# HybridRobotics/ilqr-iterative-tasks

Measured on AMD Instinct MI355X. Metric: batched iLQR iterations/s (n=6,m=2,N=20), higher is better.
Workload: dtype f64

## Files before the change

ilqr_iterative_tasks_amd/csrc/i2lqr_abi.hip:

```cpp
#include <hip/hip_runtime.h>

#include <atomic>
#include <cmath>
#include <cstdarg>
#include <cstdio>
#include <cstdlib>
#include <cstring>
#include <mutex>
#include <new>
#include <unordered_set>

#include "../../include/i2lqr.h"
#include "i2lqr_devcfg.hpp"
#include "i2lqr_geometry.hpp"
#include "i2lqr_group.h"
#include "i2lqr_handle.hpp"
#include "i2lqr_host.hpp"
#include "i2lqr_kernels.h"
#include "i2lqr_lane12.h"
#include "i2lqr_rccl.hpp"
#include "i2lqr_select.hpp"
#include "i2lqr_wave_opt.h"

#include "i2lqr_lane_launch.hpp"
// ... 499 lines not shown
  else if (!strcmp(name, "merge_inputs")) lane.opt_merge = v < 0 ? -1 : (v != 0);
  else if (!strcmp(name, "checkpoint_states")) lane.opt_ckpt = v < 0 ? -1 : (v != 0);
  else if (!strcmp(name, "stagger")) lane.opt_stagger = v;
  else if (!strcmp(name, "per_step_jacobians")) col.opt_fstep = v < 0 ? -1 : (v != 0);
  else if (!strcmp(name, "wave_tail")) lane.wave_tail = v < 0 ? -1 : (v > 65536 ? 65536 : v);
  else if (!strcmp(name, "first_chunk")) lane.opt_first_chunk = v < 1 ? -1 : (v > 1024 ? 1024 : v);
  else if (!strcmp(name, "helper_wavefront")) lane.opt_pair = v < 0 ? -1 : (v != 0);
  else if (!strcmp(name, "state_buffers")) lane.opt_two_x = v < 0 ? -1 : (v != 0);
  else if (!strcmp(name, "chunk_step")) lane.opt_chunk_step = v < 1 ? -1 : (v > 1024 ? 1024 : v);
  else if (!strcmp(name, "fused_compaction")) lane.opt_fuse = v < 0 ? -1 : (v != 0);
  else if (!strcmp(name, "final_round")) lane.opt_final_round = v < 0 ? -1 : (v > 20 ? 20 : v);
  else if (!strcmp(name, "speculate")) col.opt_spec = v < 0 ? -1 : (v != 0);
  else if (!strcmp(name, "group_workspace")) col.opt_group_ws = v < 0 ? -1 : (v != 0);
  else if (!strcmp(name, "group_overlap")) col.opt_group_overlap = v < 0 ? -1 : (v != 0);
  else if (!strcmp(name, "group_fixed_horizon")) col.opt_group_fixed = v < 0 ? -1 : (v != 0);
  else if (!strcmp(name, "debug_self_test")) {
#ifdef I2LQR_DEBUG
    unsigned long long* w = i2lqr::debug_trap_word();
    double* buf = nullptr;
    HIP_TRY(hipMalloc((void**)&buf, 8 * sizeof(double)));
    hipLaunchKernelGGL(k_debug_self_test, dim3(1), dim3(64), 0, (hipStream_t)0, buf, w);
    const int rc = debug_check(I2LQR_OK, nullptr);
    (void)hipFree(buf);
    return rc;
#else
    return fail(I2LQR_ERR_UNSUPPORTED, "\"debug_self_test\" exists in the index-checked debug build "
                "only (make -C ilqr_iterative_tasks_amd/csrc debug)");
#endif
  }
  else if (!strcmp(name, "line_search")) {
// ... 601 lines not shown
```

ilqr_iterative_tasks_amd/csrc/i2lqr_column_launch.hpp:

```cpp
#pragma once
#include <hip/hip_runtime.h>

#include "i2lqr_column_plan.hpp"
#include "i2lqr_devcfg.hpp"
#include "i2lqr_group.h"
#include "i2lqr_handle.hpp"
#include "i2lqr_host.hpp"
#include "i2lqr_kernels.h"
#include "i2lqr_wave_opt.h"

namespace i2lqr {

inline thread_local i2lqr_handle::Epilogue* t_epi = nullptr;

inline int64_t registered_ws(const i2lqr_handle* h) { return h->ws ? h->ws_bytes : -1; }
inline ColumnChoice column_kernel(const i2lqr_handle* h, int64_t B, bool early_exit) {
  return column_kernel(h->geo, h->fit, h->col, h->model.form(), registered_ws(h), B, early_exit);
}

inline int wave_lds_check(const i2lqr_handle* h, bool chained) {
  const size_t need = wave_lds_need(h->fit, h->model, chained);
  if (need <= h->geo.max_dyn_lds) return I2LQR_OK;
  const WaveForm f = h->model.form(chained);
  const int n_obs = h->model.records();
// ... 23 lines not shown
      return fail(I2LQR_ERR_UNSUPPORTED, "horizon %d needs %zu B of LDS per wavefront (> %zu KiB)",
                  h->cfg.N, lds, h->geo.max_dyn_lds / 1024);
    if (lds > h->geo.default_dyn_lds)
      for (const void* kernel :
           {(const void*)k_iterate<T, Sys, LANES, false>, (const void*)k_iterate<T, Sys, LANES, true>,
            (const void*)k_backward<T, Sys, LANES, false>, (const void*)k_backward<T, Sys, LANES, true>,
            (const void*)k_forward<T, Sys, LANES, false>, (const void*)k_forward<T, Sys, LANES, true>,
            (const void*)k_rollout<T, Sys, LANES, false>, (const void*)k_rollout<T, Sys, LANES, true>})
        HIP_TRY(hipFuncSetAttribute(kernel, hipFuncAttributeMaxDynamicSharedMemorySize, (int)lds));
    return I2LQR_OK;
  }

  static int iterate(i2lqr_handle* h, const SolveIO& io, hipStream_t s) {
    const int64_t B = io.B;
    IterArgs<T> a = iter_args<T>(io);
#ifdef I2LQR_STAMPS
    a.dbg = (unsigned long long*)h->ws;
#endif
    const ColumnChoice choice = column_kernel(h, B, io.early_exit != 0);
    const ColumnKernel fk = choice.kernel;
    if (t_epi && (fk == K_GROUP || fk == K_GROUP16 || fk == K_GROUP_WS)) {
      a.qfun = t_epi->qfun;
      a.outer_iter = t_epi->outer_iter;
      a.max_relax_iter = t_epi->max_relax_iter;
      a.cost_it = (T*)t_epi->cost_it;
      if (t_epi->best_idx) {
        a.pick_part = (MinPair<T>*)t_epi->part;
        a.pick_ticket = h->ticket + h->ticket_next.fetch_add(1, std::memory_order_relaxed) %
                                        i2lqr_handle::kTickets;
        a.best_idx = t_epi->best_idx;
// ... 62 lines not shown
        return I2LQR_OK;
      }
    }
    with_weights(c.flags, [&](auto W) {
      hipLaunchKernelGGL((k_iterate<T, Sys, LANES, W>), dim3(grid(B)), dim3(64), h->fit.lds_wave, s, c, a);
    });
    HIP_TRY(hipGetLastError());
    return I2LQR_OK;
  }
  static int names_pair(const i2lqr_handle*, int64_t, int) { return 0; }
  static int solve_chained(i2lqr_handle* h, const SolveIO& io, int k, hipStream_t s) {
    const ChainPlan plan = chain_plan(h->geo, h->fit, h->col, h->model.form(), registered_ws(h), io.B);
    if (plan.kind == ChainPlan::REFUSED) return fail(I2LQR_ERR_UNSUPPORTED, "%s", plan.why);
    IterArgs<T> a = iter_args<T>(io);
    a.chain_len = k;
    if (plan.kind == ChainPlan::WAVE) {
      if (int rc = wave_lds_check(h, true)) return rc;
      HIP_TRY(wave_opt_launch<T>(h->cfg, a, h->model, true, h->fit.lds_wave, s));
    } else if constexpr (kBicycle) {
      HIP_TRY(group_spec_chain<T>(h->cfg, a, s));
    }
    return I2LQR_OK;
  }
  static int rollout(i2lqr_handle* h, int64_t B, void* X, void* U, const void* x_term, void* cost,
                     hipStream_t s) {
    const Cfg c = make_dev_cfg<T, n, m>(h->cfg);
    with_weights(c.flags, [&](auto W) {
      hipLaunchKernelGGL((k_rollout<T, Sys, LANES, W>), dim3(grid(B)), dim3(64), h->fit.lds_wave, s, c,
                         B, (T*)X, (T*)U, (const T*)x_term, (T*)cost);
    });
// ... 30 lines not shown
```

ilqr_iterative_tasks_amd/csrc/i2lqr_column_plan.hpp:

```cpp
#pragma once
#include <cstddef>
#include <cstdint>
#include <cstdio>

#include "../../include/i2lqr.h"
#include "i2lqr_geometry.hpp"
#include "i2lqr_wave_model.hpp"

namespace i2lqr {

struct ColumnTune {
  int opt_fstep = -1;
  int opt_group = -1;
  int opt_spec = -1;
  int opt_group_ws = -1;
  int opt_group_overlap = -1;
  int opt_group_fixed = -1;
  int opt_wave_chain = 0;
};

struct ColumnFit {
  enum Plant { OTHER, BICYCLE, SIXTEEN };
  int plant = OTHER;
  bool weights = false;
  bool problem_major = false;
  bool f64 = true;
  int n = 0, N = 0, word = 8;
  bool fixed_horizon = false;
  size_t lds_wave = 0, lds_wave_fstep = 0;
  size_t lds_group8 = 0, lds_group16 = 0;
  size_t lds_group_ws = 0;
  size_t lds_spec8x2 = 0, lds_spec8x3 = 0;
// ... 243 lines not shown
```

ilqr_iterative_tasks_amd/csrc/i2lqr_dryrun.hpp:

```cpp
#pragma once
#ifdef I2LQR_DRY_RUN
#include <hip/hip_runtime.h>

#include <cstddef>
#include <cstdint>

#include "i2lqr_wave.hpp"

namespace i2lqr {
namespace dry {

bool on();
void allow(const void* base, size_t bytes);
void reset();
void record(const char* expr, const void* kernel, dim3 grid, dim3 block, size_t lds);
void ptr(const char* field, const void* p);
void val(const char* field, int64_t v);
void end();
int64_t report(char* buf, int64_t n);

template <class A> inline void arg(const A&) {}
inline void arg(int64_t v) { val("int", v); }
inline void arg(int v) { val("int", v); }
template <class P> inline void arg(P* p) { ptr("pointer argument", (const void*)p); }
// ... 4 lines not shown
  ptr("IterArgs.K", a.K); ptr("IterArgs.k", a.k); ptr("IterArgs.iters", a.iters);
  ptr("IterArgs.status", a.status); ptr("IterArgs.dbg", a.dbg); ptr("IterArgs.count", a.count);
  val("IterArgs.count_max", a.count_max); val("IterArgs.max_total", a.max_total);
  val("IterArgs.set_stride", a.set_stride);
  ptr("IterArgs.orig", a.orig); ptr("IterArgs.out_X", a.out_X);
  ptr("IterArgs.out_U", a.out_U); ptr("IterArgs.out_K", a.out_K);
  ptr("IterArgs.out_k", a.out_k); ptr("IterArgs.out_lamb", a.out_lamb);
  ptr("IterArgs.out_cost", a.out_cost); ptr("IterArgs.out_iters", a.out_iters);
  ptr("IterArgs.out_status", a.out_status);
  val("IterArgs.out_B", a.out_B); val("IterArgs.out_tiled", a.out_tiled);
  ptr("IterArgs.qfun", a.qfun);
  val("IterArgs.outer_iter", a.outer_iter); val("IterArgs.max_relax_iter", a.max_relax_iter);
  ptr("IterArgs.cost_it", a.cost_it); ptr("IterArgs.pick_part", a.pick_part);
  ptr("IterArgs.pick_ticket", a.pick_ticket); ptr("IterArgs.best_idx", a.best_idx);
  ptr("IterArgs.best_cost", a.best_cost); val("IterArgs.chain_len", a.chain_len);
}
#ifdef I2LQR_DRY_RUN_LANE
template <class T> inline void arg(const LaneSet<T>& s) {
  ptr("LaneSet.X", s.X); ptr("LaneSet.U", s.U); ptr("LaneSet.x_term", s.x_term);
  ptr("LaneSet.obs", s.obs); ptr("LaneSet.lamb", s.lamb); ptr("LaneSet.cost", s.cost);
  ptr("LaneSet.K", s.K); ptr("LaneSet.k", s.k); ptr("LaneSet.iters", s.iters);
  ptr("LaneSet.status", s.status); ptr("LaneSet.orig", s.orig); val("LaneSet.B", s.B);
}
template <class T> inline void arg(const LaneArgs<T>& a) {
  val("LaneArgs.B", a.B); val("LaneArgs.n_iters", a.n_iters); val("LaneArgs.early_exit", a.early_exit);
  ptr("LaneArgs.X", a.X); ptr("LaneArgs.U", a.U); ptr("LaneArgs.x_term", a.x_term);
  ptr("LaneArgs.lamb", a.lamb); ptr("LaneArgs.obs", a.obs); ptr("LaneArgs.cost", a.cost);
  ptr("LaneArgs.K", a.K); ptr("LaneArgs.k", a.k); ptr("LaneArgs.iters", a.iters);
  ptr("LaneArgs.status", a.status); ptr("LaneArgs.wsU", a.wsU); ptr("LaneArgs.wsK", a.wsK);
  ptr("LaneArgs.wsk", a.wsk); ptr("LaneArgs.wsX", a.wsX); ptr("LaneArgs.count", a.count);
// ... 48 lines not shown
```

ilqr_iterative_tasks_amd/csrc/i2lqr_group.hpp:

```cpp
#pragma once
#include <hip/hip_runtime.h>
#include <stdint.h>

#include "i2lqr_systems.hpp"
#include "i2lqr_wave.hpp"

namespace i2lqr {

constexpr int kGroup = 8;
constexpr int kGroupsPerWave = 64 / kGroup;

template <class Sys> struct GroupPattern {
  static constexpr int n = Sys::n, m = Sys::m, W = n + m, NV = Sys::NVAR;
  static constexpr int dt_row(int b) {
    for (int i = 2; i < n; i++)
      if (i != b && Sys::pat(i, b) == 2) return i;
    return -1;
  }
  static constexpr bool column_ok(int b) {
    int extra = 0;
    for (int i = 0; i < n; i++) {
      const int code = Sys::pat(i, b);
      if (i < 2) {
        if (code == 2) return false;
// ... 206 lines not shown
  template <int i, int a> __device__ __forceinline__ void f_acc(T& acc, bool& first, T v,
                                                                const T (&jv)[NV]) const {
    constexpr int code = Sys::pat(i, a);
    if constexpr (code == 0) {
      return;
    } else if constexpr (code == 1) {
      acc = first ? v : acc + v;
      first = false;
    } else {
      const T f = code == 2 ? c.dt : jv[code >= 3 ? code - 3 : 0];
      acc = first ? f * v : t_fma(f, v, acc);
      first = false;
    }
  }

  __device__ __forceinline__ T rollout(int XUo, int TRo, const T (&xT)[n]) const {
    T x[n], u[m], xn[n], tr[NT];
#pragma unroll
    for (int i = 0; i < n; i++) x[i] = S[XUo + i];
    const int N = loop_N();
    for (int t = 0; t < N; t++) {
#pragma unroll
      for (int a = 0; a < m; a++) u[a] = clip(S[XUo + t * W + n + a], -c.u_max[a], c.u_max[a]);
#pragma unroll
      for (int a = 0; a < m; a++) S[XUo + t * W + n + a] = u[a];
      Sys::trig(x, tr);
#pragma unroll
      for (int q = 0; q < NT; q++) S[TRo + t * NT + q] = tr[q];
      Sys::step_tr(c, x, u, tr, xn);
#pragma unroll
      for (int i = 0; i < n; i++) S[XUo + (t + 1) * W + i] = xn[i];
#pragma unroll
      for (int i = 0; i < n; i++) x[i] = xn[i];
    }
    Sys::trig(x, tr);
#pragma unroll
    for (int q = 0; q < NT; q++) S[TRo + N * NT + q] = tr[q];
    const T cost = terminal_cost(x, xT);
    wave_sync();
    return cost;
  }

  __device__ __forceinline__ void prep(int XUo, int TRo, const T (&ob)[6], T pa, T pb, int first,
                                       int stride) const {
    const bool has_ob = ob[5] >= T(0);
    const int opt = has_ob ? (int)ob[5] : 0;
    const T spd_y = opt == 1 ? ob[4] : T(0), spd_x = opt == 2 ? ob[4] : T(0);
    const int rounds = (N + stride) / stride;
    for (int r = 0; r < rounds; r++) {
      const int t0 = first + r * stride;
      const int t = t0 < N ? t0 : N;
      const int ts = t0 < N ? t0 : N - 1;
      T* Rs = rec(ts);
      {
        T xe[n], tr[NT], u[m], jv[NV];
#pragma unroll
        for (int i = 0; i < n; i++) xe[i] = S[XUo + (ts + 1) * W + i];
#pragma unroll
        for (int a = 0; a < m; a++) u[a] = S[XUo + ts * W + n + a];
// ... 21 lines not shown
      R[GL::R_ZERO] = T(0);
      R[GL::R_ONE] = T(1);
      const T px = S[XUo + t * W + 0], py = S[XUo + t * W + 1];
      const T dz = opt == 2 ? px - (ob[0] - T(t) * spd_x) : px - ob[0];
      const T dy = opt == 1 ? py - (ob[1] + T(t) * spd_y) : py - ob[1];
      const T h = T(1) + c.safety_margin - (dz * pa * dz + dy * pb * dy);
      const T hd0 = T(-2) * pa * dz, hd1 = T(-2) * pb * dy;
      const T e = t_exp(c.obs_q2 * h);
      const T c1 = c.obs_q12 * e, c2 = c.obs_q122 * e;
      R[GL::R_OB + 0] = has_ob ? c1 * hd0 : T(0);
      R[GL::R_OB + 1] = has_ob ? c1 * hd1 : T(0);
      R[GL::R_OB + 2] = has_ob ? c2 * (hd0 * hd0) : T(0);
      R[GL::R_OB + 3] = has_ob ? c2 * (hd0 * hd1) : T(0);
      R[GL::R_OB + 4] = has_ob ? c2 * (hd1 * hd1) : T(0);
    }
    wave_sync();
    ws_publish();
  }

  __device__ __forceinline__ void quu_inverse(const T (&Quu)[m * m], T lamb, T (&inv)[m * m]) const {
    static_assert(m == 2, "the eight-lane kernel is written for m == 2 plants");
    t_quu_inverse2(Quu, lamb, inv);
  }

  template <bool GENERAL>
  __device__ __forceinline__ bool backward(int XUo, const T (&xT)[n], T lamb, bool commit) const {
    if constexpr (G == 16) return backward_row<GENERAL>(XUo, xT, lamb, commit);
    bool bad = false;
    T va[n];
    {
      const T* Rn = rec(N);
      T dx[n];
// ... 346 lines not shown
          step(t - 3, rb, ra);
        }
      }
      for (; t >= 1; t -= 2) {
        step(t, ra, rb);
        step(t - 1, rb, ra);
      }
      if (t == 0) step(0, ra, rb);
    }
    STAMP_END(1);
    wave_sync();
    return bad;
  }

  __device__ __forceinline__ T forward_row(int XUo, int XUn, int TRn, const T (&xT)[n],
                                           bool* bad) const {
    static_assert(G == 16 && m == 2, "two inputs on the two halves of a 16-lane row");
    const int half = g >> 3;
    const T umax = half ? c.u_max[1] : c.u_max[0];
    T x[n], u[m], xn[n], tr[NT];
#pragma unroll
    for (int i = 0; i < n; i++) x[i] = S[XUo + i];
#pragma unroll
    for (int i = 0; i < n; i++) S[XUn + i] = x[i];
    Sys::template trig_g<false>(x, tr, bad);
#pragma unroll
    for (int q = 0; q < NT; q++) S[TRn + q] = tr[q];
    static_assert(!WS, "gain rows and records are neighbours in the LDS slice");
    auto pXo = S + XUo;
    auto pXn = S + XUn;
    auto pG = S + (oKk + half * GL::KW);
    auto pTR = S + (TRn + half * NT);
    T xo[n], uo, kk[NA];
    auto load_step = [&](auto k_) __attribute__((always_inline)) {
      constexpr int k = decltype(k_)::value;
#pragma unroll
      for (int j = 0; j < n; j++) xo[j] = pXo[k * W + j];
      uo = pXo[k * W + n + half];
#pragma unroll
      for (int j = 0; j < NA; j++) kk[j] = pG[k * (m * GL::KW) + j];
// ... 42 lines not shown
      if constexpr (NH % 2 != 0) I2LQR_FORWARD_ROW_LAST()
    } else {
      int t = 0;
      for (; t + 1 < N; t += 2) I2LQR_FORWARD_ROW_PAIR()
      if (t < N) I2LQR_FORWARD_ROW_LAST()
    }
#undef I2LQR_FORWARD_ROW_PAIR
#undef I2LQR_FORWARD_ROW_LAST
    const T cost = terminal_cost(x, xT);
    wave_sync();
    return cost;
  }

  template <bool GENERAL>
  __device__ __forceinline__ T forward(int XUo, int XUn, int TRn, const T (&xT)[n],
                                       bool* bad) const {
    if constexpr (G == 16 && !GENERAL && Sys::kHeadingAhead && m == 2)
      return forward_row(XUo, XUn, TRn, xT, bad);
    const int N = loop_N();
    T x[n], u[m], xn[n], tr[NT];
#pragma unroll
    for (int i = 0; i < n; i++) x[i] = S[XUo + i];
#pragma unroll
    for (int i = 0; i < n; i++) S[XUn + i] = x[i];
    T xo[n], uo[m];
    struct Gains { T kk[m][NA]; };
    Gains ga, gb;
    auto load_gains = [&](int t, Gains& q) __attribute__((always_inline)) {
      const T* Kg = gain(t);
#pragma unroll
      for (int a = 0; a < m; a++)
#pragma unroll
        for (int j = 0; j < NA; j++) q.kk[a][j] = Kg[a * GL::KW + j];
// ... 120 lines not shown
  T lamb = a.lamb[prob];
  wave_sync();

  int cur = 0;
  const T ob_pa = T(1) / (ob[2] * ob[2]), ob_pb = T(1) / (ob[3] * ob[3]);
  int* const ctl = reinterpret_cast<int*>(smem + L.ctl_base());
  if constexpr (H > 1) {
    if (hv > 0) {
      const int h0 = OVL ? hv - 1 : hv, hs = OVL ? H - 1 : H;
      for (;;) {
        __syncthreads();
        const int flags = ctl[8];
        if (!(flags & 1)) break;
        if (flags & 2) {
          const int pc = ctl[lane / G];
          w.prep(pc ? L.XU1 : L.XU0, pc ? L.TR1 : L.TR0, ob, ob_pa, ob_pb, h0 * G + g, hs * G);
        }
        __syncthreads();
      }
      if constexpr (OVL) {
        if (real && a.K) {
          T* const gK = a.K + prob * (int64_t)(m * n * N);
          T* const gk = a.k + prob * (int64_t)(m * N);
          for (int t = h0 * G + g; t < N; t += hs * G) {
            const T* Kt = w.gain(t);
            T kv[m][n + 1];
#pragma unroll
            for (int aa = 0; aa < m; aa++)
#pragma unroll
              for (int j = 0; j <= n; j++) kv[aa][j] = Kt[aa * GL::KW + j];
#pragma unroll
            for (int aa = 0; aa < m; aa++) {
#pragma unroll
              for (int j = 0; j < n; j++) gK[(aa * n + j) * N + t] = kv[aa][j];
              gk[aa * N + t] = kv[aa][n];
            }
          }
        }
      }
      return;
    }
  }
  T vb[n];
#pragma unroll
  for (int i = 0; i < n; i++) vb[i] = T(0);
  T cost = w.rollout(L.XU0, L.TR0, xT);
  int it = 0, status = a.early_exit ? 2  : 0 ;
  T cost_ret = cost;
  bool fresh = true, active = a.n_iters > 0;
#ifdef I2LQR_STAMPS
  asm volatile("s_memtime %0\n\ts_waitcnt lgkmcnt(0)" : "=s"(st_k1)::"memory");
#endif
  while (__any(active)) {
    const int XUo = cur ? L.XU1 : L.XU0, XUn = cur ? L.XU0 : L.XU1;
    const int TRo = cur ? L.TR1 : L.TR0, TRn = cur ? L.TR0 : L.TR1;
#ifdef I2LQR_STAMPS
    {
      auto& st_t0 = w.st_t0; auto& st_t1 = w.st_t1; auto& st_acc = w.st_acc;
      STAMP_BEGIN();
      if (__any(fresh)) w.prep(XUo, TRo, ob, ob_pa, ob_pb, g, G);
      STAMP_END(0);
    }
#else
    if constexpr (H > 1) {
      const bool do_prep = __any(fresh);
      if (g == 0) ctl[lane / G] = cur;
      if (lane == 0) ctl[8] = 1 | (do_prep ? 2 : 0);
      __syncthreads();
      if constexpr (OVL) {
        if (do_prep) w.terminal_base(XUo, xT, vb);
      } else {
        if (do_prep) w.prep(XUo, TRo, ob, ob_pa, ob_pb, g, H * G);
      }
      __syncthreads();
    } else {
      if (__any(fresh)) w.prep(XUo, TRo, ob, ob_pa, ob_pb, g, G);
    }
#endif
    if constexpr (OVL) {
      if (__builtin_expect(__any(w.template backward_row_from<false>(vb, lamb, active)), 0))
        w.template backward_row_from<true>(vb, lamb, active);
    } else {
      if (__builtin_expect(__any(w.template backward<false>(XUo, xT, lamb, active)), 0))
        w.template backward<true>(XUo, xT, lamb, active);
    }
    T cost_new;
    {
#ifdef I2LQR_STAMPS
      auto& st_t0 = w.st_t0; auto& st_t1 = w.st_t1; auto& st_acc = w.st_acc;
      STAMP_BEGIN();
#endif
      bool big = false;
      cost_new = w.template forward<false>(XUo, XUn, TRn, xT, &big);
      if (__builtin_expect(__any(big), 0)) cost_new = w.template forward<true>(XUo, XUn, TRn, xT, &big);
#ifdef I2LQR_STAMPS
      STAMP_END(6);
#endif
    }
    {
      const bool acc = active && cost_new < cost, rej = active && !(cost_new < cost);
      const T lamb_dn = lamb / c.lamb_factor, lamb_up = lamb * c.lamb_factor;
      const bool conv = t_abs((cost_new - cost) / cost) < c.eps;
      it += active ? 1 : 0;
      fresh = acc;
      cur ^= acc ? 1 : 0;
      lamb = acc ? lamb_dn : (rej ? lamb_up : lamb);
      cost_ret = acc ? cost_new : (rej ? cost : cost_ret);
      cost = acc ? cost_new : cost;
// ... 187 lines not shown
    }
    for (int e = lane; e < n * n; e += 64) QtL[e] = c.Qt[e];
  }
  T xT[n], ob[6];
#pragma unroll
  for (int i = 0; i < n; i++) xT[i] = SETIO ? a.x_term[i * Bs + prob] : a.x_term[prob * n + i];
#pragma unroll
  for (int q = 0; q < 6; q++)
    ob[q] = a.obs ? (SETIO ? a.obs[q * Bs + prob] : a.obs[prob * 6 + q]) : T(q == 5 ? -1 : 1);
  T lamb = (CHAIN && cstep > 0) ? lamb_carry : a.lamb[prob];
  const int it0 = SETIO ? a.iters[prob] : 0;
  const int it_cap = SETIO ? a.max_total - it0 : a.n_iters;
  const T ob_pa = T(1) / (ob[2] * ob[2]), ob_pb = T(1) / (ob[3] * ob[3]);
  __syncthreads();
  if (v == 0) {
    const T c0 = w.rollout(SLay.xu_off(0), SLay.tr_off(0), xT);
    if (g == 0) CN[V * PW + p] = c0;
  }
  __syncthreads();
  T cost = CN[V * PW + p];

  int nb = 0, cb[V];
#pragma unroll
  for (int k = 0; k < V; k++) cb[k] = k + 1;
  int it = 0, status = a.early_exit ? 2  : 0 , gsel = 0;
  T cost_ret = cost;
  bool fresh = true, active = it_cap > 0;
  while (__any(active)) {
    if (__any(fresh)) {
      w.prep(SLay.xu_off(nb), SLay.tr_off(nb), ob, ob_pa, ob_pb, v * G + g, V * G);
      __syncthreads();
    }
    T lamb_v = lamb;
    for (int k = 0; k < v; k++) lamb_v *= c.lamb_factor;
    int mycb = cb[0];
#pragma unroll
    for (int k = 1; k < V; k++) mycb = (v == k) ? cb[k] : mycb;
    const int XUo = SLay.xu_off(nb), XUn = SLay.xu_off(mycb), TRn = SLay.tr_off(mycb);
    if (__builtin_expect(__any(w.template backward<false>(XUo, xT, lamb_v, active)), 0))
      w.template backward<true>(XUo, xT, lamb_v, active);
    bool big = false;
    T cost_new = w.template forward<false>(XUo, XUn, TRn, xT, &big);
    if (__builtin_expect(__any(big), 0)) cost_new = w.template forward<true>(XUo, XUn, TRn, xT, &big);
    if (g == 0) CN[v * PW + p] = cost_new;
    __syncthreads();
    fresh = false;
    bool chain = active;
#pragma unroll
    for (int k = 0; k < V; k++) {
      if (chain) {
        const T cn = CN[k * PW + p];
        it++;
        gsel = k;
        if (cn < cost) {
          const int tb = nb; nb = cb[k]; cb[k] = tb;
          lamb /= c.lamb_factor;
          const bool conv = t_abs((cn - cost) / cost) < c.eps;
// ... 106 lines not shown
```

ilqr_iterative_tasks_amd/csrc/i2lqr_systems.hpp:

```cpp
#pragma once
#include <hip/hip_runtime.h>

#include <type_traits>

namespace i2lqr {

template <class T> __device__ __forceinline__ void t_sincos(T x, T* s, T* c);
template <bool SLIT, unsigned long long BITS>
__device__ __forceinline__ double t_lit_at(double dep) {
  if constexpr (SLIT) {
    unsigned lo, hi;
    asm volatile("s_mov_b32 %0, %2\n\ts_mov_b32 %1, %3"
                 : "=s"(lo), "=s"(hi)
                 : "n"((unsigned)(BITS & 0xffffffffull)), "n"((unsigned)(BITS >> 32)), "v"(dep));
    return __builtin_bit_cast(double, ((unsigned long long)hi << 32) | lo);
  } else {
    return __builtin_bit_cast(double, BITS);
  }
}
#define I2LQR_LIT(SLIT, value, dep) \
  t_lit_at<SLIT, __builtin_bit_cast(unsigned long long, (double)(value))>(dep)
template <class T> __device__ __forceinline__ void t_sincos_fast(T x, T* s, T* c, bool* big_out);
template <bool SLIT, int NS>
__device__ __forceinline__ void t_sincos_fast_dn(const double (&x)[NS], double (&s)[NS],
// ... 56 lines not shown
template <bool SLIT>
__device__ __forceinline__ void t_sincos_fast_d(double x, double* s, double* c, bool* big_out) {
  const double xa[1] = {x};
  double sa[1], ca[1];
  t_sincos_fast_dn<SLIT, 1>(xa, sa, ca, big_out);
  *s = sa[0];
  *c = ca[0];
}
template <> __device__ __forceinline__ void t_sincos_fast<double>(double x, double* s, double* c,
                                                                   bool* big_out) {
  t_sincos_fast_d<false>(x, s, c, big_out);
}
__device__ __forceinline__ double t_fma3(double a, double b, double c) {
  double d;
  asm("v_fma_f64 %0, %1, %2, %3" : "=v"(d) : "v"(a), "v"(b), "v"(c));
  return d;
}
__device__ __forceinline__ void t_sincos_fast_h3(double x, double* s, double* c, bool* big_out) {
  const bool big = !(__builtin_fabs(x) < 1.0e5);
  *big_out = *big_out || big;
  const double xs = big ? 0.0 : x;
  const double kf = __builtin_rint(xs * 6.36619772367581382433e-01);
  double r = __builtin_fma(-kf, 1.57079632679489655800e+00, xs);
  r = __builtin_fma(-kf, 6.12323399573676603587e-17, r);
  r = __builtin_fma(-kf, -1.49738490485916983327e-33, r);
  const double z = r * r;
  double ps = 1.58969099521155010221e-10, pc = -1.13596475577881948265e-11;
#define I2LQR_SC_STEP3(ls, lc) \
  ps = t_fma3(ps, z, ls);      \
  pc = t_fma3(pc, z, lc);
// ... 53 lines not shown
}
template <> __device__ __forceinline__ void t_sincos<float>(float x, float* s, float* c) {
  bool big = false;
  float so, co;
  t_sincos_fast(x, &so, &co, &big);
  if (__builtin_expect(__any(big), 0)) {
    float sl, cl;
    sincosf(x, &sl, &cl);
    so = big ? sl : so;
    co = big ? cl : co;
  }
  *s = so;
  *c = co;
}
template <class T> __device__ __forceinline__ T t_exp(T x);
template <bool SLIT, int NE, int NB>
__device__ __forceinline__ void t_exp_d(const double (&x0)[NE], double (&e)[NE]) {
  double x[NE], kf[NE], r[NE], p[NE];
#pragma unroll
  for (int q = 0; q < NE; q++)
    x[q] = q < NE - NB ? (x0[q] < I2LQR_LIT(SLIT, -746.0, x0[q]) ? -746.0
                          : (x0[q] > I2LQR_LIT(SLIT, 710.0, x0[q]) ? 710.0 : x0[q]))
                       : x0[q];
  const double l2e = I2LQR_LIT(SLIT, 1.44269504088896338700e+00, x[0]);
#pragma unroll
  for (int q = 0; q < NE; q++) kf[q] = __builtin_rint(x[q] * l2e);
  const double ln2h = I2LQR_LIT(SLIT, 6.93147180369123816490e-01, kf[0]);
#pragma unroll
  for (int q = 0; q < NE; q++) r[q] = __builtin_fma(-kf[q], ln2h, x[q]);
  const double ln2l = I2LQR_LIT(SLIT, 1.90821492927058770002e-10, r[0]);
#pragma unroll
  for (int q = 0; q < NE; q++) r[q] = __builtin_fma(-kf[q], ln2l, r[q]);
  const double c13 = I2LQR_LIT(SLIT, 1.6059043836821614599e-10, r[0]);
#pragma unroll
  for (int q = 0; q < NE; q++) p[q] = c13;
#define I2LQR_EXP_STEP(lit)                                          \
  {                                                                  \
    const double ck = I2LQR_LIT(SLIT, lit, p[0]);                    \
    _Pragma("unroll") for (int q = 0; q < NE; q++) p[q] = __builtin_fma(p[q], r[q], ck); \
  }
  I2LQR_EXP_STEP(2.0876756987868098979e-09)
  I2LQR_EXP_STEP(2.5052108385441718775e-08)
  I2LQR_EXP_STEP(2.7557319223985890653e-07)
  I2LQR_EXP_STEP(2.7557319223985892511e-06)
  I2LQR_EXP_STEP(2.4801587301587301566e-05)
  I2LQR_EXP_STEP(1.9841269841269841253e-04)
  I2LQR_EXP_STEP(1.3888888888888889419e-03)
  I2LQR_EXP_STEP(8.3333333333333332177e-03)
  I2LQR_EXP_STEP(4.1666666666666664354e-02)
  I2LQR_EXP_STEP(1.6666666666666665741e-01)
#undef I2LQR_EXP_STEP
#pragma unroll
  for (int q = 0; q < NE; q++) {
    p[q] = __builtin_fma(p[q], r[q], 0.5);
// ... 28 lines not shown
template <> __device__ __forceinline__ double t_fma<double>(double a, double b, double c) {
  return __builtin_fma(a, b, c);
}
template <> __device__ __forceinline__ float t_fma<float>(float a, float b, float c) {
  return __builtin_fmaf(a, b, c);
}

template <class T> __device__ __forceinline__ T t_rcp(T x);
template <> __device__ __forceinline__ double t_rcp<double>(double x) {
  double r = __builtin_amdgcn_rcp(x);
  double e = __builtin_fma(-x, r, 1.0);
  r = __builtin_fma(r, e, r);
  e = __builtin_fma(-x, r, 1.0);
  const double r2 = __builtin_fma(r, e, r);
  return (r2 == r2) ? r2 : r;
}
template <> __device__ __forceinline__ float t_rcp<float>(float x) {
  const float r = __builtin_amdgcn_rcpf(x);
  const float e = __builtin_fmaf(-x, r, 1.0f);
  const float r2 = __builtin_fmaf(r, e, r);
  return (r2 == r2) ? r2 : r;
}
template <class T> __device__ __forceinline__ T t_sqrt_fast(T x);
template <> __device__ __forceinline__ double t_sqrt_fast<double>(double x) {
  if (!(x > 1.0e-290) || !(x < 1.0e290)) return __builtin_sqrt(x);
  const double y = __builtin_amdgcn_rsq(x);
  double g = x * y;
  double h = 0.5 * y;
  double r = __builtin_fma(-h, g, 0.5);
  g = __builtin_fma(g, r, g);
// ... 243 lines not shown
    }
#pragma unroll
    for (int e = 0; e < m * m; e++) inv[e] = pd ? inv[e] : ginv[e];
  }
}

template <class T> struct Bicycle4 {
  static constexpr int n = 4, m = 2, NTRIG = 2, NVAR = 6;
  static constexpr int NCONST = 0, NBLK = 0;
  static constexpr int NJX = 0;
  static constexpr int jx(int) { return 0; }
  static constexpr int blk(int) { return 0; }
  template <class Cfg> static __device__ __forceinline__ T plant_const(const Cfg&, int) { return T(0); }
  static constexpr int system_id = 0;
  static constexpr bool kHeadingAhead = false;

  static __device__ __forceinline__ void trig(const T (&xe)[n], T (&tr)[NTRIG]) {
    t_sincos(xe[3], &tr[1], &tr[0]);
  }
  template <bool GENERAL>
  static __device__ __forceinline__ void trig_g(const T (&xe)[n], T (&tr)[NTRIG], bool* bad) {
    if constexpr (GENERAL) t_sincos(xe[3], &tr[1], &tr[0]);
    else t_sincos_fast(xe[3], &tr[1], &tr[0], bad);
  }
  template <class Cfg>
  static __device__ __forceinline__ void step_tr(const Cfg& c, const T (&x)[n], const T (&u)[m],
                                                 const T (&tr)[NTRIG], T (&xn)[n]) {
    const T dt = c.dt;
    const T w = x[2] * dt + (u[0] * dt * dt) / T(2);
    xn[0] = x[0] + tr[0] * w;
// ... 39 lines not shown
  template <class Cfg> static __device__ __forceinline__ T jac_const(const Cfg& c, int i, int j) {
    if (j < n) return (i == j) ? T(1) : T(0);
    return ((i == 2 && j == n) || (i == 3 && j == n + 1)) ? c.dt : T(0);
  }
};

template <class T> struct Bicycle6 {
  static constexpr int n = 6, m = 2, NTRIG = 2, NVAR = 6;
  static constexpr int NCONST = 0, NBLK = 0;
  static constexpr int NJX = 0;
  static constexpr int jx(int) { return 0; }
  static constexpr int blk(int) { return 0; }
  template <class Cfg> static __device__ __forceinline__ T plant_const(const Cfg&, int) { return T(0); }
  static constexpr int system_id = 1;
  static constexpr bool kHeadingAhead = true;
  static __device__ __forceinline__ T heading(const T (&xe)[n]) { return xe[3]; }
  template <class Cfg>
  static __device__ __forceinline__ T next_heading(const Cfg& c, const T (&xe)[n]) {
    return xe[3] + xe[5] * c.dt;
  }
  static __device__ __forceinline__ void trig_heading_fast(T ang, T (&tr)[NTRIG], bool* bad) {
    t_sincos_fast_h3(ang, &tr[1], &tr[0], bad);
  }

  static __device__ __forceinline__ void trig(const T (&xe)[n], T (&tr)[NTRIG]) {
    t_sincos(xe[3], &tr[1], &tr[0]);
  }
  template <bool GENERAL>
  static __device__ __forceinline__ void trig_g(const T (&xe)[n], T (&tr)[NTRIG], bool* bad) {
    if constexpr (GENERAL) t_sincos(xe[3], &tr[1], &tr[0]);
// ... 49 lines not shown
  }
  template <class Cfg> static __device__ __forceinline__ T jac_const(const Cfg& c, int i, int j) {
    if (j < n) {
      if (i == j) return T(1);
      return ((i == 2 && j == 4) || (i == 3 && j == 5)) ? c.dt : T(0);
    }
    return ((i == 4 && j == n) || (i == 5 && j == n + 1)) ? c.dt : T(0);
  }
};

template <class T> struct Quad12 {
  static constexpr int n = 12, m = 4, NTRIG = 6;
  static constexpr int NVAR = 37;
  static constexpr int system_id = 2;
  static constexpr bool kHeadingAhead = false;

  static __device__ __forceinline__ void trig(const T (&xe)[n], T (&tr)[NTRIG]) {
    t_sincos(xe[3], &tr[0], &tr[1]);
    t_sincos(xe[4], &tr[2], &tr[3]);
    t_sincos(xe[5], &tr[4], &tr[5]);
  }
  template <bool GENERAL>
  static __device__ __forceinline__ void trig_g(const T (&xe)[n], T (&tr)[NTRIG], bool* bad) {
    if constexpr (GENERAL) {
      trig(xe, tr);
    } else {
      t_sincos_fast(xe[3], &tr[0], &tr[1], bad);
      t_sincos_fast(xe[4], &tr[2], &tr[3], bad);
      t_sincos_fast(xe[5], &tr[4], &tr[5], bad);
    }
// ... 164 lines not shown
```

ilqr_iterative_tasks_amd/csrc/i2lqr_wave.hpp:

```cpp
#pragma once
#include <hip/hip_runtime.h>
#include <stdint.h>

#include <type_traits>

#include "i2lqr_debug.hpp"
#include "i2lqr_systems.hpp"


namespace i2lqr {

enum : int { FLAG_HAS_Q = 1, FLAG_HAS_R = 2 };

template <class T, int n, int m> struct DevCfg {
  int N, max_iter, flags;
  int fast_barrier;
  T dt, eps, lamb_factor, max_lamb;
  T ctrl_q1, ctrl_q2, obs_q1, obs_q2, safety_margin;
  T u_max[m];
  T ctrl_c[m];
  T xtarget[n];
  T Q[n * n], Qt[n * n], R[m * m];
  T sys_par[8];
  T ctrl_q12, ctrl_q122, obs_q12, obs_q122;
// ... 36 lines not shown
  T* out_k = nullptr;
  T* out_lamb = nullptr;
  T* out_cost = nullptr;
  int32_t* out_iters = nullptr;
  int32_t* out_status = nullptr;
  int64_t out_B = 0;
  int out_tiled = 0;
  const int32_t* qfun = nullptr;
  int outer_iter = 0, max_relax_iter = 0;
  T* cost_it = nullptr;
  MinPair<T>* pick_part = nullptr;
  unsigned* pick_ticket = nullptr;
  int64_t* best_idx = nullptr;
  T* best_cost = nullptr;
  int chain_len = 1;
};

__device__ __forceinline__ double relax_cost_value(double ss, int32_t qf, int N, int outer_iter,
                                                   int max_relax_iter) {
  const double nrm = sqrt(ss);
  double scale = 1.0;
  for (int q = 0; q < outer_iter; q++) scale *= 10.0;
  double out = INFINITY;
  if (qf == 0x7fffffff) return out;
  for (int i = 1; i <= max_relax_iter; i++) {
    if (nrm <= 80.0 * i / scale) { out = (double)qf + N + 100 * i; break; }
    if (nrm > 80.0 * max_relax_iter / scale) break;
  }
  return out;
}
// ... 852 lines not shown
```

Measured before the change: 82.15 million.

## Add chained group prep and rollout that reuse stored trig values

Adds a 'group_chains' path for the 16-lane group kernels. The initial rollout is split into a clip pass, a serial integration of the trig-free state tail, a parallel trig pass and a final serial pass. The cost-record prep computes its exponentials with a fused multi-exp using scalar-operand FMAs and a paired reciprocal to replace the lower-bound exps. The forward pass reads the x0 trig from LDS instead of recomputing it. The aim is to move transcendental work off the serial critical path, at the cost of extra LDS traffic, extra wave syncs and more code.

```diff
diff --git a/ilqr_iterative_tasks_amd/csrc/i2lqr_abi.hip b/ilqr_iterative_tasks_amd/csrc/i2lqr_abi.hip
--- a/ilqr_iterative_tasks_amd/csrc/i2lqr_abi.hip
+++ b/ilqr_iterative_tasks_amd/csrc/i2lqr_abi.hip
@@ -537,6 +537,7 @@
   else if (!strcmp(name, "group_workspace")) col.opt_group_ws = v < 0 ? -1 : (v != 0);
   else if (!strcmp(name, "group_overlap")) col.opt_group_overlap = v < 0 ? -1 : (v != 0);
   else if (!strcmp(name, "group_fixed_horizon")) col.opt_group_fixed = v < 0 ? -1 : (v != 0);
+  else if (!strcmp(name, "group_chains")) col.opt_group_chains = v < 0 ? -1 : (v != 0);
   else if (!strcmp(name, "debug_self_test")) {
 #ifdef I2LQR_DEBUG
     unsigned long long* w = i2lqr::debug_trap_word();
diff --git a/ilqr_iterative_tasks_amd/csrc/i2lqr_column_launch.hpp b/ilqr_iterative_tasks_amd/csrc/i2lqr_column_launch.hpp
--- a/ilqr_iterative_tasks_amd/csrc/i2lqr_column_launch.hpp
+++ b/ilqr_iterative_tasks_amd/csrc/i2lqr_column_launch.hpp
@@ -61,6 +61,7 @@
   static int iterate(i2lqr_handle* h, const SolveIO& io, hipStream_t s) {
     const int64_t B = io.B;
     IterArgs<T> a = iter_args<T>(io);
+    a.chains = h->col.opt_group_chains != 0;
 #ifdef I2LQR_STAMPS
     a.dbg = (unsigned long long*)h->ws;
 #endif
@@ -153,6 +154,7 @@
     if (plan.kind == ChainPlan::REFUSED) return fail(I2LQR_ERR_UNSUPPORTED, "%s", plan.why);
     IterArgs<T> a = iter_args<T>(io);
     a.chain_len = k;
+    a.chains = h->col.opt_group_chains != 0;
     if (plan.kind == ChainPlan::WAVE) {
       if (int rc = wave_lds_check(h, true)) return rc;
       HIP_TRY(wave_opt_launch<T>(h->cfg, a, h->model, true, h->fit.lds_wave, s));
diff --git a/ilqr_iterative_tasks_amd/csrc/i2lqr_column_plan.hpp b/ilqr_iterative_tasks_amd/csrc/i2lqr_column_plan.hpp
--- a/ilqr_iterative_tasks_amd/csrc/i2lqr_column_plan.hpp
+++ b/ilqr_iterative_tasks_amd/csrc/i2lqr_column_plan.hpp
@@ -16,6 +16,7 @@
   int opt_group_ws = -1;
   int opt_group_overlap = -1;
   int opt_group_fixed = -1;
+  int opt_group_chains = -1;
   int opt_wave_chain = 0;
 };
 
diff --git a/ilqr_iterative_tasks_amd/csrc/i2lqr_dryrun.hpp b/ilqr_iterative_tasks_amd/csrc/i2lqr_dryrun.hpp
--- a/ilqr_iterative_tasks_amd/csrc/i2lqr_dryrun.hpp
+++ b/ilqr_iterative_tasks_amd/csrc/i2lqr_dryrun.hpp
@@ -42,6 +42,7 @@
   ptr("IterArgs.cost_it", a.cost_it); ptr("IterArgs.pick_part", a.pick_part);
   ptr("IterArgs.pick_ticket", a.pick_ticket); ptr("IterArgs.best_idx", a.best_idx);
   ptr("IterArgs.best_cost", a.best_cost); val("IterArgs.chain_len", a.chain_len);
+  val("IterArgs.chains", a.chains);
 }
 #ifdef I2LQR_DRY_RUN_LANE
 template <class T> inline void arg(const LaneSet<T>& s) {
diff --git a/ilqr_iterative_tasks_amd/csrc/i2lqr_group.hpp b/ilqr_iterative_tasks_amd/csrc/i2lqr_group.hpp
--- a/ilqr_iterative_tasks_amd/csrc/i2lqr_group.hpp
+++ b/ilqr_iterative_tasks_amd/csrc/i2lqr_group.hpp
@@ -244,7 +244,10 @@
     }
   }
 
-  __device__ __forceinline__ T rollout(int XUo, int TRo, const T (&xT)[n]) const {
+  __device__ __forceinline__ T rollout(int XUo, int TRo, const T (&xT)[n], bool chains) const {
+    if constexpr (G == 16 && Sys::kTrigFreeTail) {
+      if (__builtin_expect(chains, 1)) return rollout_row(XUo, TRo, xT);
+    }
     T x[n], u[m], xn[n], tr[NT];
 #pragma unroll
     for (int i = 0; i < n; i++) x[i] = S[XUo + i];
@@ -271,8 +274,171 @@
     return cost;
   }
 
+  __device__ __forceinline__ T rollout_row(int XUo, int TRo, const T (&xT)[n]) const {
+    static_assert(G == 16 && Sys::kTrigFreeTail, "see Sys::kTrigFreeTail");
+    const int N = loop_N();
+    for (int t = g; t < N; t += G) {
+      T u[m];
+#pragma unroll
+      for (int a = 0; a < m; a++) u[a] = clip(S[XUo + t * W + n + a], -c.u_max[a], c.u_max[a]);
+#pragma unroll
+      for (int a = 0; a < m; a++) S[XUo + t * W + n + a] = u[a];
+    }
+    wave_sync();
+    T x[n], u[m], xn[n], tr[NT];
+#pragma unroll
+    for (int i = 0; i < n; i++) x[i] = S[XUo + i];
+#pragma unroll
+    for (int q = 0; q < NT; q++) tr[q] = T(0);
+    for (int t = 0; t < N; t++) {
+#pragma unroll
+      for (int a = 0; a < m; a++) u[a] = S[XUo + t * W + n + a];
+      Sys::step_tr(c, x, u, tr, xn);
+#pragma unroll
+      for (int i = 2; i < n; i++) S[XUo + (t + 1) * W + i] = xn[i];
+#pragma unroll
+      for (int i = 2; i < n; i++) x[i] = xn[i];
+    }
+    const int rounds = (N + G) / G;
+    for (int r = 0; r < rounds; r++) {
+      const int t0 = g + r * G;
+      const int t = t0 < N ? t0 : N;
+      T xe[n];
+      xe[0] = T(0); xe[1] = T(0);
+#pragma unroll
+      for (int i = 2; i < n; i++) xe[i] = S[XUo + t * W + i];
+      Sys::trig(xe, tr);
+#pragma unroll
+      for (int q = 0; q < NT; q++) S[TRo + t * NT + q] = tr[q];
+    }
+    wave_sync();
+    T un[m], trn[NT];
+#pragma unroll
+    for (int i = 0; i < n; i++) x[i] = S[XUo + i];
+#pragma unroll
+    for (int a = 0; a < m; a++) u[a] = S[XUo + n + a];
+#pragma unroll
+    for (int q = 0; q < NT; q++) tr[q] = S[TRo + q];
+    for (int t = 0; t < N; t++) {
+#pragma unroll
+      for (int a = 0; a < m; a++) un[a] = S[XUo + (t + 1) * W + n + a];
+#pragma unroll
+      for (int q = 0; q < NT; q++) trn[q] = S[TRo + (t + 1) * NT + q];
+      Sys::step_tr(c, x, u, tr, xn);
+#pragma unroll
+      for (int i = 0; i < n; i++) S[XUo + (t + 1) * W + i] = xn[i];
+#pragma unroll
+      for (int i = 0; i < n; i++) x[i] = xn[i];
+#pragma unroll
+      for (int a = 0; a < m; a++) u[a] = un[a];
+#pragma unroll
+      for (int q = 0; q < NT; q++) tr[q] = trn[q];
+    }
+    const T cost = terminal_cost(x, xT);
+    wave_sync();
+    return cost;
+  }
+
   __device__ __forceinline__ void prep(int XUo, int TRo, const T (&ob)[6], T pa, T pb, int first,
-                                       int stride) const {
+                                       int stride, bool chains) const {
+    if (__builtin_expect(chains, 1)) {
+      if (sizeof(T) == 8 && __builtin_expect(c.fast_barrier, 1))
+        prep_chains<true>(XUo, TRo, ob, pa, pb, first, stride);
+      else
+        prep_chains<false>(XUo, TRo, ob, pa, pb, first, stride);
+    } else {
+      prep_serial(XUo, TRo, ob, pa, pb, first, stride);
+    }
+    wave_sync();
+    ws_publish();
+  }
+
+  template <bool FASTB>
+  __device__ __forceinline__ void prep_chains(int XUo, int TRo, const T (&ob)[6], T pa, T pb,
+                                              int first, int stride) const {
+    static_assert(m == 2, "two inputs");
+    const bool has_ob = ob[5] >= T(0);
+    const int opt = has_ob ? (int)ob[5] : 0;
+    const T spd_y = opt == 1 ? ob[4] : T(0), spd_x = opt == 2 ? ob[4] : T(0);
+    const int rounds = (N + stride) / stride;
+    for (int r = 0; r < rounds; r++) {
+      const int t0 = first + r * stride;
+      const int t = t0 < N ? t0 : N;
+      const int ts = t0 < N ? t0 : N - 1;
+      T* Rs = rec(ts);
+      T* R = rec(t);
+      if constexpr (FASTB) asm volatile("; record, short input barrier" ::: "memory");
+      else asm volatile("; record, general input barrier" ::: "memory");
+      T xe[n], tr[NT], u[m], jv[NV];
+#pragma unroll
+      for (int i = 0; i < n; i++) xe[i] = S[XUo + (ts + 1) * W + i];
+#pragma unroll
+      for (int a = 0; a < m; a++) u[a] = S[XUo + ts * W + n + a];
+#pragma unroll
+      for (int q = 0; q < NT; q++) tr[q] = S[TRo + (ts + 1) * NT + q];
+      const T px = S[XUo + t * W + 0], py = S[XUo + t * W + 1];
+      const T dz = opt == 2 ? px - (ob[0] - T(t) * spd_x) : px - ob[0];
+      const T dy = opt == 1 ? py - (ob[1] + T(t) * spd_y) : py - ob[1];
+      const T h = T(1) + c.safety_margin - (dz * pa * dz + dy * pb * dy);
+      const T hd0 = T(-2) * pa * dz, hd1 = T(-2) * pb * dy;
+      T e, e_hi[m], e_lo[m];
+      if constexpr (FASTB) {
+        const double xa[3] = {(double)(c.obs_q2 * h), (double)(c.ctrl_q2 * (u[0] - c.u_max[0])),
+                              (double)(c.ctrl_q2 * (u[1] - c.u_max[1]))};
+        double ea[3], rc[2];
+        t_exp_d<false, 3, 2, true>(xa, ea);
+        t_rcp2(ea[1], ea[2], &rc[0], &rc[1]);
+        e = (T)ea[0];
+#pragma unroll
+        for (int a = 0; a < m; a++) {
+          e_hi[a] = (T)ea[1 + a];
+          e_lo[a] = c.ctrl_c[a] * (T)rc[a];
+        }
+      } else if constexpr (sizeof(T) == 8) {
+        const double xa[5] = {(double)(c.obs_q2 * h), (double)(c.ctrl_q2 * (u[0] - c.u_max[0])),
+                              (double)(c.ctrl_q2 * (-c.u_max[0] - u[0])),
+                              (double)(c.ctrl_q2 * (u[1] - c.u_max[1])),
+                              (double)(c.ctrl_q2 * (-c.u_max[1] - u[1]))};
+        double ea[5];
+        t_exp_d<false, 5, 0, true>(xa, ea);
+        e = (T)ea[0];
+#pragma unroll
+        for (int a = 0; a < m; a++) {
+          e_hi[a] = (T)ea[1 + 2 * a];
+          e_lo[a] = (T)ea[2 + 2 * a];
+        }
+      } else {
+        e = t_exp(c.obs_q2 * h);
+#pragma unroll
+        for (int a = 0; a < m; a++) {
+          e_hi[a] = t_exp(c.ctrl_q2 * (u[a] - c.u_max[a]));
+          e_lo[a] = t_exp(c.ctrl_q2 * (-c.u_max[a] - u[a]));
+        }
+      }
+      Sys::jac_var(c, xe, u, tr, jv);
+#pragma unroll
+      for (int q = 0; q < NV; q++) Rs[GL::R_JV + q] = jv[q];
+#pragma unroll
+      for (int a = 0; a < m; a++) {
+        Rs[GL::R_LU + a] = c.ctrl_q12 * e_hi[a] - c.ctrl_q12 * e_lo[a];
+        Rs[GL::R_LUU + a] = c.ctrl_q122 * e_hi[a] +
+                            c.ctrl_q122 * e_lo[a];
+      }
+      R[GL::R_ZERO] = T(0);
+      R[GL::R_ONE] = T(1);
+      const T c1 = c.obs_q12 * e, c2 = c.obs_q122 * e;
+      R[GL::R_OB + 0] = has_ob ? c1 * hd0 : T(0);
+      R[GL::R_OB + 1] = has_ob ? c1 * hd1 : T(0);
+      R[GL::R_OB + 2] = has_ob ? c2 * (hd0 * hd0) : T(0);
+      R[GL::R_OB + 3] = has_ob ? c2 * (hd0 * hd1) : T(0);
+      R[GL::R_OB + 4] = has_ob ? c2 * (hd1 * hd1) : T(0);
+      if constexpr (FASTB) asm volatile("; record end, short input barrier" ::: "memory");
+      else asm volatile("; record end, general input barrier" ::: "memory");
+    }
+  }
+
+  __device__ __forceinline__ void prep_serial(int XUo, int TRo, const T (&ob)[6], T pa, T pb,
+                                              int first, int stride) const {
     const bool has_ob = ob[5] >= T(0);
     const int opt = has_ob ? (int)ob[5] : 0;
     const T spd_y = opt == 1 ? ob[4] : T(0), spd_x = opt == 2 ? ob[4] : T(0);
@@ -324,8 +490,6 @@
       R[GL::R_OB + 3] = has_ob ? c2 * (hd0 * hd1) : T(0);
       R[GL::R_OB + 4] = has_ob ? c2 * (hd1 * hd1) : T(0);
     }
-    wave_sync();
-    ws_publish();
   }
 
   __device__ __forceinline__ void quu_inverse(const T (&Quu)[m * m], T lamb, T (&inv)[m * m]) const {
@@ -702,7 +866,7 @@
   }
 
   __device__ __forceinline__ T forward_row(int XUo, int XUn, int TRn, const T (&xT)[n],
-                                           bool* bad) const {
+                                           bool* bad, bool chains, int TRo) const {
     static_assert(G == 16 && m == 2, "two inputs on the two halves of a 16-lane row");
     const int half = g >> 3;
     const T umax = half ? c.u_max[1] : c.u_max[0];
@@ -711,7 +875,15 @@
     for (int i = 0; i < n; i++) x[i] = S[XUo + i];
 #pragma unroll
     for (int i = 0; i < n; i++) S[XUn + i] = x[i];
-    Sys::template trig_g<false>(x, tr, bad);
+#ifdef I2LQR_FORWARD_X0_TRIG
+    chains = false;
+#endif
+    if (__builtin_expect(chains, 1)) {
+#pragma unroll
+      for (int q = 0; q < NT; q++) tr[q] = S[TRo + q];
+    } else {
+      Sys::template trig_g<false>(x, tr, bad);
+    }
 #pragma unroll
     for (int q = 0; q < NT; q++) S[TRn + q] = tr[q];
     static_assert(!WS, "gain rows and records are neighbours in the LDS slice");
@@ -784,9 +956,9 @@
 
   template <bool GENERAL>
   __device__ __forceinline__ T forward(int XUo, int XUn, int TRn, const T (&xT)[n],
-                                       bool* bad) const {
+                                       bool* bad, bool chains = false, int TRo = 0) const {
     if constexpr (G == 16 && !GENERAL && Sys::kHeadingAhead && m == 2)
-      return forward_row(XUo, XUn, TRn, xT, bad);
+      return forward_row(XUo, XUn, TRn, xT, bad, chains, TRo);
     const int N = loop_N();
     T x[n], u[m], xn[n], tr[NT];
 #pragma unroll
@@ -937,7 +1109,8 @@
         if (!(flags & 1)) break;
         if (flags & 2) {
           const int pc = ctl[lane / G];
-          w.prep(pc ? L.XU1 : L.XU0, pc ? L.TR1 : L.TR0, ob, ob_pa, ob_pb, h0 * G + g, hs * G);
+          w.prep(pc ? L.XU1 : L.XU0, pc ? L.TR1 : L.TR0, ob, ob_pa, ob_pb, h0 * G + g, hs * G,
+                 a.chains != 0);
         }
         __syncthreads();
       }
@@ -967,7 +1140,8 @@
   T vb[n];
 #pragma unroll
   for (int i = 0; i < n; i++) vb[i] = T(0);
-  T cost = w.rollout(L.XU0, L.TR0, xT);
+  const bool chains = a.chains != 0;
+  T cost = w.rollout(L.XU0, L.TR0, xT, chains);
   int it = 0, status = a.early_exit ? 2  : 0 ;
   T cost_ret = cost;
   bool fresh = true, active = a.n_iters > 0;
@@ -981,7 +1155,7 @@
     {
       auto& st_t0 = w.st_t0; auto& st_t1 = w.st_t1; auto& st_acc = w.st_acc;
       STAMP_BEGIN();
-      if (__any(fresh)) w.prep(XUo, TRo, ob, ob_pa, ob_pb, g, G);
+      if (__any(fresh)) w.prep(XUo, TRo, ob, ob_pa, ob_pb, g, G, chains);
       STAMP_END(0);
     }
 #else
@@ -993,11 +1167,11 @@
       if constexpr (OVL) {
         if (do_prep) w.terminal_base(XUo, xT, vb);
       } else {
-        if (do_prep) w.prep(XUo, TRo, ob, ob_pa, ob_pb, g, H * G);
+        if (do_prep) w.prep(XUo, TRo, ob, ob_pa, ob_pb, g, H * G, chains);
       }
       __syncthreads();
     } else {
-      if (__any(fresh)) w.prep(XUo, TRo, ob, ob_pa, ob_pb, g, G);
+      if (__any(fresh)) w.prep(XUo, TRo, ob, ob_pa, ob_pb, g, G, chains);
     }
 #endif
     if constexpr (OVL) {
@@ -1014,7 +1188,7 @@
       STAMP_BEGIN();
 #endif
       bool big = false;
-      cost_new = w.template forward<false>(XUo, XUn, TRn, xT, &big);
+      cost_new = w.template forward<false>(XUo, XUn, TRn, xT, &big, chains, TRo);
       if (__builtin_expect(__any(big), 0)) cost_new = w.template forward<true>(XUo, XUn, TRn, xT, &big);
 #ifdef I2LQR_STAMPS
       STAMP_END(6);
@@ -1232,7 +1406,7 @@
   const T ob_pa = T(1) / (ob[2] * ob[2]), ob_pb = T(1) / (ob[3] * ob[3]);
   __syncthreads();
   if (v == 0) {
-    const T c0 = w.rollout(SLay.xu_off(0), SLay.tr_off(0), xT);
+    const T c0 = w.rollout(SLay.xu_off(0), SLay.tr_off(0), xT, a.chains != 0);
     if (g == 0) CN[V * PW + p] = c0;
   }
   __syncthreads();
@@ -1246,7 +1420,7 @@
   bool fresh = true, active = it_cap > 0;
   while (__any(active)) {
     if (__any(fresh)) {
-      w.prep(SLay.xu_off(nb), SLay.tr_off(nb), ob, ob_pa, ob_pb, v * G + g, V * G);
+      w.prep(SLay.xu_off(nb), SLay.tr_off(nb), ob, ob_pa, ob_pb, v * G + g, V * G, a.chains != 0);
       __syncthreads();
     }
     T lamb_v = lamb;
@@ -1258,7 +1432,7 @@
     if (__builtin_expect(__any(w.template backward<false>(XUo, xT, lamb_v, active)), 0))
       w.template backward<true>(XUo, xT, lamb_v, active);
     bool big = false;
-    T cost_new = w.template forward<false>(XUo, XUn, TRn, xT, &big);
+    T cost_new = w.template forward<false>(XUo, XUn, TRn, xT, &big, a.chains != 0, SLay.tr_off(nb));
     if (__builtin_expect(__any(big), 0)) cost_new = w.template forward<true>(XUo, XUn, TRn, xT, &big);
     if (g == 0) CN[v * PW + p] = cost_new;
     __syncthreads();
diff --git a/ilqr_iterative_tasks_amd/csrc/i2lqr_systems.hpp b/ilqr_iterative_tasks_amd/csrc/i2lqr_systems.hpp
--- a/ilqr_iterative_tasks_amd/csrc/i2lqr_systems.hpp
+++ b/ilqr_iterative_tasks_amd/csrc/i2lqr_systems.hpp
@@ -94,6 +94,11 @@
 __device__ __forceinline__ double t_fma3(double a, double b, double c) {
   double d;
   asm("v_fma_f64 %0, %1, %2, %3" : "=v"(d) : "v"(a), "v"(b), "v"(c));
+  return d;
+}
+__device__ __forceinline__ double t_fma3s(double a, double b, double c) {
+  double d;
+  asm("v_fma_f64 %0, %1, %2, %3" : "=v"(d) : "v"(a), "v"(b), "s"(c));
   return d;
 }
 __device__ __forceinline__ void t_sincos_fast_h3(double x, double* s, double* c, bool* big_out) {
@@ -177,11 +182,16 @@
   *c = co;
 }
 template <class T> __device__ __forceinline__ T t_exp(T x);
-template <bool SLIT, int NE, int NB>
+template <bool SLIT, int NE, int NB, bool H3 = false>
 __device__ __forceinline__ void t_exp_d(const double (&x0)[NE], double (&e)[NE]) {
+  static_assert(!(SLIT && H3), "the three-address form takes its coefficients from vector registers");
   double x[NE], kf[NE], r[NE], p[NE];
 #pragma unroll
   for (int q = 0; q < NE; q++)
+    if constexpr (H3) {
+      const double lo = x0[q] < -746.0 ? -746.0 : x0[q];
+      x[q] = q < NE - NB ? (lo > 710.0 ? 710.0 : lo) : x0[q];
+    } else
     x[q] = q < NE - NB ? (x0[q] < I2LQR_LIT(SLIT, -746.0, x0[q]) ? -746.0
                           : (x0[q] > I2LQR_LIT(SLIT, 710.0, x0[q]) ? 710.0 : x0[q]))
                        : x0[q];
@@ -200,7 +210,8 @@
 #define I2LQR_EXP_STEP(lit)                                          \
   {                                                                  \
     const double ck = I2LQR_LIT(SLIT, lit, p[0]);                    \
-    _Pragma("unroll") for (int q = 0; q < NE; q++) p[q] = __builtin_fma(p[q], r[q], ck); \
+    _Pragma("unroll") for (int q = 0; q < NE; q++)                   \
+      p[q] = H3 ? t_fma3s(p[q], r[q], ck) : __builtin_fma(p[q], r[q], ck); \
   }
   I2LQR_EXP_STEP(2.0876756987868098979e-09)
   I2LQR_EXP_STEP(2.5052108385441718775e-08)
@@ -259,6 +270,20 @@
   e = __builtin_fma(-x, r, 1.0);
   const double r2 = __builtin_fma(r, e, r);
   return (r2 == r2) ? r2 : r;
+}
+__device__ __forceinline__ void t_rcp2(double x0, double x1, double* o0, double* o1) {
+  double r0 = __builtin_amdgcn_rcp(x0);
+  double r1 = __builtin_amdgcn_rcp(x1);
+  double e0 = __builtin_fma(-x0, r0, 1.0);
+  double e1 = __builtin_fma(-x1, r1, 1.0);
+  r0 = __builtin_fma(r0, e0, r0);
+  r1 = __builtin_fma(r1, e1, r1);
+  e0 = __builtin_fma(-x0, r0, 1.0);
+  e1 = __builtin_fma(-x1, r1, 1.0);
+  const double q0 = __builtin_fma(r0, e0, r0);
+  const double q1 = __builtin_fma(r1, e1, r1);
+  *o0 = (q0 == q0) ? q0 : r0;
+  *o1 = (q1 == q1) ? q1 : r1;
 }
 template <> __device__ __forceinline__ float t_rcp<float>(float x) {
   const float r = __builtin_amdgcn_rcpf(x);
@@ -532,6 +557,7 @@
   template <class Cfg> static __device__ __forceinline__ T plant_const(const Cfg&, int) { return T(0); }
   static constexpr int system_id = 0;
   static constexpr bool kHeadingAhead = false;
+  static constexpr bool kTrigFreeTail = true;
 
   static __device__ __forceinline__ void trig(const T (&xe)[n], T (&tr)[NTRIG]) {
     t_sincos(xe[3], &tr[1], &tr[0]);
@@ -601,6 +627,7 @@
   template <class Cfg> static __device__ __forceinline__ T plant_const(const Cfg&, int) { return T(0); }
   static constexpr int system_id = 1;
   static constexpr bool kHeadingAhead = true;
+  static constexpr bool kTrigFreeTail = true;
   static __device__ __forceinline__ T heading(const T (&xe)[n]) { return xe[3]; }
   template <class Cfg>
   static __device__ __forceinline__ T next_heading(const Cfg& c, const T (&xe)[n]) {
@@ -680,6 +707,7 @@
   static constexpr int NVAR = 37;
   static constexpr int system_id = 2;
   static constexpr bool kHeadingAhead = false;
+  static constexpr bool kTrigFreeTail = false;
 
   static __device__ __forceinline__ void trig(const T (&xe)[n], T (&tr)[NTRIG]) {
     t_sincos(xe[3], &tr[0], &tr[1]);
diff --git a/ilqr_iterative_tasks_amd/csrc/i2lqr_wave.hpp b/ilqr_iterative_tasks_amd/csrc/i2lqr_wave.hpp
--- a/ilqr_iterative_tasks_amd/csrc/i2lqr_wave.hpp
+++ b/ilqr_iterative_tasks_amd/csrc/i2lqr_wave.hpp
@@ -74,6 +74,7 @@
   int64_t* best_idx = nullptr;
   T* best_cost = nullptr;
   int chain_len = 1;
+  int chains = 1;
 };
 
 __device__ __forceinline__ double relax_cost_value(double ss, int32_t qf, int N, int outer_iter,
```

Result: faster. 84.19 million (median of 6 runs) (+2.5%).
